# 1275468127/Medical-SAM2

Measured on AMD Instinct MI355X. Metric: slices/sec @1024^2 (Hiera-S), higher is better.
Workload: dtype bf16; 1 GPU; configs[1]: sam2_hiera_s 2D (train_2d SAM2 sub-sequence, forward), b=4 x 1024x1024 per GPU, 16-entry memory bank with 4 sampled memories per slice, one click per slice; forward_image -> memory_attention -> prompt encoder -> mask decoder -> memory encoder; hip_graph=True, weights=random name-keyed init

## Files before the change

include/msam2_hip.h:

```cpp
#ifndef MSAM2_HIP_H
#define MSAM2_HIP_H

#include <stddef.h>
#include <stdint.h>

#ifdef __cplusplus
extern "C" {
#endif

const char* msam2_last_error(void);

int msam2_version(void);

int msam2_operand_is_fp16(void);

int msam2_graph_begin(void* stream);

int msam2_graph_end(void* stream, void** graph_exec_out);

int msam2_graph_launch(void* graph_exec, void* stream);

int msam2_graph_destroy(void* graph_exec);

int msam2_event_create(void** ev);
// ... 185 lines not shown
int msam2_ln_mlp_residual_fwd(const float* x, int64_t T, int64_t dim, const float* ln_w, const float* ln_b, float eps, const void* w1, const float* b1, const void* w2p, const float* b2, float* out, void* stream);

int msam2_ln_mlp_residual_fwd_dual(const float* x, int64_t T, int64_t dim, const float* ln_w, const float* ln_b, float eps, const void* w1, const float* b1, const void* w2p, const float* b2, float* out, void* out16, void* stream);

size_t msam2_mask_stats_workspace_bytes(int64_t M);

int msam2_mask_stats(const float* logits, int64_t M, int64_t lh, int64_t lw, int64_t h, int64_t w, float thr, float thr_hi, float thr_lo, int* counts, int* boxes, void* workspace, size_t workspace_bytes, void* stream);

int msam2_mask_rle_runs(const float* logits, int64_t M, int64_t lh, int64_t lw, int64_t h, int64_t w, int64_t x0, int64_t y0, int64_t H, int64_t W, float thr, int* runs, void* stream);

int msam2_mask_rle(const float* logits, int64_t M, int64_t lh, int64_t lw, int64_t h, int64_t w, int64_t x0, int64_t y0, int64_t H, int64_t W, float thr, const int64_t* offsets, int* counts, void* stream);

size_t msam2_box_nms_workspace_bytes(int64_t K);

int msam2_box_nms(const float* boxes, const float* scores, int64_t K, float iou_thr, int64_t* keep, int* n_keep, void* workspace, size_t workspace_bytes, void* stream);

#ifdef __cplusplus
}
#endif
#endif
```

medical-sam2_amd/_lib.py:

```python
from __future__ import annotations

import ctypes
import os
import subprocess

_HERE = os.path.dirname(os.path.abspath(__file__))
LIB_PATH = os.environ.get("MSAM2_LIB_PATH") or os.path.join(_HERE, "libmsam2_hip.so")

c_p = ctypes.c_void_p
c_i = ctypes.c_int
c_l = ctypes.c_int64
c_f = ctypes.c_float
c_z = ctypes.c_size_t

SIGNATURES = {
    "msam2_version": (c_i, []),
    "msam2_last_error": (ctypes.c_char_p, []),
    "msam2_operand_is_fp16": (c_i, []),
    "msam2_gemm": (c_i, [c_p, c_l, c_p, c_l, c_p, c_p, c_p, c_l, c_i, c_l, c_p, c_l, c_i, c_l, c_l, c_l, c_i, c_p]),
    "msam2_gemm_pool2x2": (c_i, [c_p, c_l, c_p, c_l, c_p, c_p, c_l, c_l, c_l, c_l, c_l, c_l, c_p]),
    "msam2_gemm_qkv_pool2x2": (c_i, [c_p, c_l, c_p, c_l, c_p, c_p, c_l, c_p, c_l, c_l, c_l, c_l, c_l, c_l, c_l, c_p]),
    "msam2_gemm_tokens": (c_i, [c_p, c_l, c_p, c_l, c_p, c_l, c_p, c_p, c_l, c_p, c_l, c_i, c_l, c_l, c_l, c_i, c_p]),
    "msam2_gemm_rope": (c_i, [c_p, c_l, c_p, c_l, c_p, c_p, c_l, c_l, c_l, c_l, c_p, c_p, c_l, c_l, c_l, c_l, c_l, c_p]),
    "msam2_ln_mlp_residual_supported": (c_i, [c_l]),
# ... 89 lines not shown
    "msam2_box_nms": (c_i, [c_p, c_p, c_l, c_f, c_p, c_p, c_p, c_z, c_p]),
    "msam2_cc_workspace_bytes": (c_z, [c_l, c_l, c_l]),
    "msam2_cc_label": (c_i, [c_p, c_p, c_p, c_l, c_l, c_l, c_p, c_z, c_p]),
    "msam2_fill_holes_workspace_bytes": (c_z, [c_l, c_l, c_l]),
    "msam2_fill_holes": (c_i, [c_p, c_l, c_l, c_l, c_i, c_p, c_z, c_p]),
    "msam2_fill_components": (c_i, [c_p, c_l, c_l, c_l, c_i, c_f, c_i, c_f, c_p, c_z, c_p]),
    "msam2_image_prep": (c_i, [c_p, c_p, c_l, c_l, c_l, ctypes.POINTER(c_f), ctypes.POINTER(c_f), c_p]),
    "msam2_graph_begin": (c_i, [c_p]),
    "msam2_graph_end": (c_i, [c_p, ctypes.POINTER(c_p)]),
    "msam2_graph_launch": (c_i, [c_p, c_p]),
    "msam2_graph_destroy": (c_i, [c_p]),
    "msam2_event_create": (c_i, [ctypes.POINTER(c_p)]),
    "msam2_event_record": (c_i, [c_p, c_p]),
    "msam2_event_elapsed_ms": (c_i, [c_p, c_p, ctypes.POINTER(c_f)]),
    "msam2_event_destroy": (c_i, [c_p]),
}


def build(force: bool = False) -> str:
    if force and os.path.exists(LIB_PATH):
        os.remove(LIB_PATH)
    subprocess.check_call(["make", "-s", "-C", os.path.join(_HERE, "csrc")])
    return LIB_PATH


_lib = None


def lib() -> ctypes.CDLL:
    global _lib
# ... 22 lines not shown
```

medical-sam2_amd/modeling/common.py:

```python
from __future__ import annotations

from typing import Callable, Dict, Sequence, Tuple

import torch

from .. import ops

OP16, F32 = ops.OP16, torch.float32


class WeightCache:

    def __init__(self):
        self._c: Dict[str, Tuple[tuple, object]] = {}
        self._casts: Dict[str, torch.Tensor] = {}

    @staticmethod
    def _sig(params: Sequence[torch.Tensor]) -> tuple:
        return tuple((p.data_ptr(), p._version, str(p.device), p.dtype) for p in params)

    def get(self, key: str, params: Sequence[torch.Tensor], build: Callable[[], object], cast_of: torch.Tensor = None):
        sig = self._sig(params)
        hit = self._c.get(key)
        if hit is None or hit[0] != sig:
# ... 101 lines not shown
```

medical-sam2_amd/modeling/encoder.py:

```python
from __future__ import annotations

from typing import List, Optional, Tuple

import torch
import torch.nn as nn

from .. import ops
from .common import OP16, F32, WeightCache, nchw_view, to_bf16, tokens_of, v_f32, w_bf16
from .position import PositionEmbeddingSine


import os as _os
_POOL_GEMM = _os.environ.get("MSAM2_NO_POOL_GEMM") is None
_QPOOL_GEMM = _os.environ.get("MSAM2_NO_QPOOL_GEMM") is None
_FUSED_MLP = _os.environ.get("MSAM2_NO_FUSED_MLP") is None
_FUSED_PATCH = _os.environ.get("MSAM2_NO_FUSED_PATCH") is None


class PatchEmbed(nn.Module):

    def __init__(self, kernel_size=(7, 7), stride=(4, 4), padding=(3, 3), in_chans: int = 3, embed_dim: int = 768):
        super().__init__()
        assert tuple(kernel_size) == (7, 7) and tuple(stride) == (4, 4) and tuple(padding) == (3, 3) and in_chans == 3, \
            "the HIP path implements the 7x7/4/3 RGB patch embedding used by every SAM2 config"
# ... 126 lines not shown
            out = torch.zeros(3, heads, Dp, dtype=F32, device=b.device)
            out[:, :, :D] = b
            return out.reshape(-1).contiguous()

        def proj_w():
            w = a.proj.weight.detach().reshape(dim_out, heads, D)
            out = torch.zeros(dim_out, heads, Dp, dtype=w.dtype, device=w.device)
            out[:, :, :D] = w
            return out.reshape(dim_out, heads * Dp).to(OP16).contiguous()

        if Dp == D:
            return D, Dp, w_bf16(wc, "qkvw", a.qkv.weight), v_f32(wc, "qkvb", a.qkv.bias), w_bf16(wc, "ow", a.proj.weight)
        return (D, Dp, wc.get("qkvw_p", [a.qkv.weight], qkv_w), wc.get("qkvb_p", [a.qkv.bias], qkv_b),
                wc.get("ow_p", [a.proj.weight], proj_w))

    def run(self, t: torch.Tensor, B: int, H: int, W: int, emit16: bool = False) -> Tuple[torch.Tensor, int, int]:
        self.out16 = None
        wc, a = self._wc, self.attn
        heads, dim_out = a.num_heads, self.dim_out
        D, Dp, qkv_w, qkv_b, proj_w = self._packed_attn_weights()
        width = heads * Dp
        scale = 1.0 / (D ** 0.5)
        xn = ops.layernorm(t, v_f32(wc, "n1w", self.norm1.weight), v_f32(wc, "n1b", self.norm1.bias), 1e-6)
        pool = self.q_stride is not None
        if self.dim != dim_out:
            if _POOL_GEMM and pool and B * H * W >= 256 and H % 2 == 0 and W % 2 == 0:
                shortcut = ops.gemm_pool2x2(xn, w_bf16(wc, "pw", self.proj.weight), v_f32(wc, "pb", self.proj.bias), B, H, W)
            else:
                shortcut = ops.gemm(xn, w_bf16(wc, "pw", self.proj.weight), v_f32(wc, "pb", self.proj.bias), out_dtype=F32)
                if pool:
                    shortcut = ops.maxpool2x2(shortcut, B, H, W)
        else:
            shortcut = t
        if _POOL_GEMM and _QPOOL_GEMM and pool and B * H * W >= 256 and H % 2 == 0 and W % 2 == 0 and width % 32 == 0:
            qkv, qp = ops.gemm_qkv_pool2x2(xn, qkv_w, qkv_b, B, H, W, width)
        else:
            qkv = ops.gemm(xn, qkv_w, qkv_b)
            qp = ops.maxpool2x2(qkv[:, :width], B, H, W) if pool else None
        Hq, Wq = (H // 2, W // 2) if pool else (H, W)
        if self.window_size > 0:
            o = ops.window_attention(qkv, B, H, W, heads, self.window_size, qkv_b, q_pooled=qp, scale=scale)
        else:
            v5 = qkv.view(B, H * W, 3, heads, Dp)
            q = (qp.view(B, Hq * Wq, heads, Dp) if pool else v5[:, :, 0]).permute(0, 2, 1, 3)
            o = ops.attention(q, v5[:, :, 1].permute(0, 2, 1, 3), v5[:, :, 2].permute(0, 2, 1, 3), scale=scale)
            o = o.permute(0, 2, 1, 3).reshape(B * Hq * Wq, width)
        t = ops.gemm(o, proj_w, v_f32(wc, "ob", a.proj.bias), residual=shortcut, out_dtype=F32)
        mlp = self.mlp
        if (_FUSED_MLP and ops.ln_mlp_residual_supported(dim_out) and mlp.num_layers == 2 and mlp._act_code == ops.ACT_GELU
                and mlp.layers[0].out_features == 4 * dim_out and Hq * Wq >= 1024):
            w2p = mlp._wc.get("w1p", [mlp.layers[1].weight], lambda: ops.mlp_fused_permute_w2(mlp.layers[1].weight.detach().to(OP16).contiguous()))
            t = ops.ln_mlp_residual(t, v_f32(wc, "n2w", self.norm2.weight), v_f32(wc, "n2b", self.norm2.bias), 1e-6,
                                    w_bf16(mlp._wc, "w0", mlp.layers[0].weight), v_f32(mlp._wc, "b0", mlp.layers[0].bias), w2p,
                                    v_f32(mlp._wc, "b1", mlp.layers[1].bias), also16=emit16)
            if emit16:
                t, self.out16 = t
            return t, Hq, Wq
        xn2 = ops.layernorm(t, v_f32(wc, "n2w", self.norm2.weight), v_f32(wc, "n2b", self.norm2.bias), 1e-6)
        t = self.mlp.run(xn2, residual=t, out_dtype=F32)
        return t, Hq, Wq

    def forward(self, x: torch.Tensor) -> torch.Tensor:
        B, H, W, C = x.shape
        t, h, w = self.run(x.to(F32).reshape(B * H * W, C).contiguous(), B, H, W)
        return t.reshape(B, h, w, -1)


class Hiera(nn.Module):

    def __init__(self, embed_dim: int = 96, num_heads: int = 1, drop_path_rate: float = 0.0, q_pool: int = 3,
                 q_stride: Tuple[int, int] = (2, 2), stages: Tuple[int, ...] = (2, 3, 16, 3), dim_mul: float = 2.0,
                 head_mul: float = 2.0, window_pos_embed_bkg_spatial_size: Tuple[int, int] = (14, 14),
                 window_spec: Tuple[int, ...] = (8, 4, 14, 7), global_att_blocks: Tuple[int, ...] = (12, 16, 20),
                 return_interm_layers=True):
        super().__init__()
# ... 28 lines not shown
        self._wc = WeightCache()

    def _pos_tokens(self, h: int, w: int) -> torch.Tensor:
        return self._wc.get(f"pos{h}x{w}", [self.pos_embed, self.pos_embed_window],
                            lambda: ops.hiera_pos_embed(self.pos_embed.detach().float(), self.pos_embed_window.detach().float(), h, w))

    def _get_pos_embed(self, hw: Tuple[int, int]) -> torch.Tensor:
        h, w = hw
        return self._pos_tokens(h, w).reshape(1, h, w, -1)

    def forward(self, x: torch.Tensor) -> List[torch.Tensor]:
        B, _, S, _ = x.shape
        h = w = S // 4
        t = self.patch_embed.tokens(x, self._pos_tokens(h, w))
        outputs = []
        for i, blk in enumerate(self.blocks):
            is_out = i == self.stage_ends[-1] or (i in self.stage_ends and self.return_interm_layers)
            t, h, w = blk.run(t, B, h, w, emit16=is_out)
            if is_out:
                v = nchw_view(t, B, h, w)
                v._op16_tokens, blk.out16 = blk.out16, None
                outputs.append(v)
        return outputs


class FpnNeck(nn.Module):

    def __init__(self, position_encoding: nn.Module, d_model: int, backbone_channel_list: List[int], kernel_size: int = 1,
                 stride: int = 1, padding: int = 0, fpn_interp_model: str = "bilinear", fuse_type: str = "sum",
                 fpn_top_down_levels: Optional[List[int]] = None):
        super().__init__()
        assert kernel_size == 1 and stride == 1 and padding == 0, "lateral convs are 1x1 in every SAM2 config"
        assert fpn_interp_model == "nearest" and fuse_type == "sum", "HIP path implements the YAML's nearest/sum top-down fusion"
# ... 60 lines not shown
```

medical-sam2_amd/modeling/memory.py:

```python
from __future__ import annotations

import copy
import math
from typing import Optional, Tuple

import torch
import torch.nn as nn

from .. import ops
from .common import OP16, F32, WeightCache, attn_splits, nchw_view, to_bf16, tokens_of, v_f32, w_bf16
from .encoder import MLP


import os as _os
_FUSED_ROPE = _os.environ.get("MSAM2_NO_FUSED_ROPE") is None
_FOLD_V = _os.environ.get("MSAM2_NO_VALUE_FOLD") is None
_BATCH_K_PROJ = _os.environ.get("MSAM2_BATCHED_KPROJ") is not None


class LayerNorm2d(nn.Module):

    def __init__(self, num_channels: int, eps: float = 1e-6) -> None:
        super().__init__()
        self.weight = nn.Parameter(torch.ones(num_channels))
        self.bias = nn.Parameter(torch.zeros(num_channels))
# ... 13 lines not shown
        self.kv_in_dim = kv_in_dim if kv_in_dim is not None else embedding_dim
        self.internal_dim = embedding_dim // downsample_rate
        self.num_heads = num_heads
        assert self.internal_dim % num_heads == 0, "num_heads must divide embedding_dim."
        self.q_proj = nn.Linear(embedding_dim, self.internal_dim)
        self.k_proj = nn.Linear(self.kv_in_dim, self.internal_dim)
        self.v_proj = nn.Linear(self.kv_in_dim, self.internal_dim)
        self.out_proj = nn.Linear(self.internal_dim, embedding_dim)
        self.dropout_p = dropout
        self._wc = WeightCache()

    def proj(self, which: str, x_bf16: torch.Tensor) -> torch.Tensor:
        lin = getattr(self, which + "_proj")
        return ops.gemm(x_bf16, w_bf16(self._wc, which + "w", lin.weight), v_f32(self._wc, which + "b", lin.bias))

    def out(self, o_bf16: torch.Tensor, residual: Optional[torch.Tensor], out_dtype=F32) -> torch.Tensor:
        return ops.gemm(o_bf16, w_bf16(self._wc, "ow", self.out_proj.weight), v_f32(self._wc, "ob", self.out_proj.bias),
                        residual=residual, out_dtype=out_dtype)

    def core(self, q: torch.Tensor, k: torch.Tensor, v: torch.Tensor) -> torch.Tensor:
        B, Lq, C = q.shape
        D = C // self.num_heads
        if D in (16, 32):
            return ops.attention_small(q, k, v, self.num_heads).reshape(B * Lq, C)
        H = self.num_heads
        sp = lambda t: t.view(B, t.shape[1], H, D).permute(0, 2, 1, 3)
        o = ops.attention(sp(q), sp(k), sp(v), splits=attn_splits(B, H, Lq, k.shape[1]))
        return o.permute(0, 2, 1, 3).reshape(B * Lq, C)

    def forward(self, q: torch.Tensor, k: torch.Tensor, v: torch.Tensor) -> torch.Tensor:
        assert not (self.training and self.dropout_p > 0.0), "attention dropout (train mode) is outside the forward hot path"
        B, Lq, _ = q.shape
        f = lambda t, n: self.proj(n, to_bf16(t.reshape(-1, t.shape[-1]).contiguous())).view(B, t.shape[1], -1)
# ... 35 lines not shown
        tiles_total = -(-valid_keys // 32)
        tiles_per = -(-tiles_total // eff)
        k0 = min(share[0] * tiles_per * 32, valid_keys)
        k1 = min(share[1] * tiles_per * 32, valid_keys)
        r0, r1 = (k0 // n_pos) * n_pos, min(-(-k1 // n_pos) * n_pos, Nk)
        kk = torch.empty(B, Nk, self.internal_dim, dtype=OP16, device=mem_k.device)
        if r1 > r0:
            n_rope = max(0, min(Nk - n_ptr_tokens, r1) - r0)
            for b in range(B):
                self.proj_rope("k", mem_k[b, r0:r1], 1, r1 - r0, n_rope, tab, out=kk[b, r0:r1])
        return kk

    def folds_values(self) -> bool:
        return _FOLD_V and self.kv_in_dim == 64 and self.internal_dim == 256 and self.num_heads == 1

    def out_folded(self, o64: torch.Tensor, residual: Optional[torch.Tensor], out_dtype=F32) -> torch.Tensor:
        ps = [self.out_proj.weight, self.out_proj.bias, self.v_proj.weight, self.v_proj.bias]
        w = self._wc.get("ovw", ps, lambda: (self.out_proj.weight.detach().float() @ self.v_proj.weight.detach().float()).to(OP16).contiguous())
        b = self._wc.get("ovb", ps, lambda: (self.out_proj.weight.detach().float() @ self.v_proj.bias.detach().float()
                                             + self.out_proj.bias.detach().float()).contiguous())
        return ops.gemm(o64, w, b, residual=residual, out_dtype=out_dtype)

    def core_folded(self, q: torch.Tensor, k: torch.Tensor, mem_v: torch.Tensor, key_count: Optional[torch.Tensor] = None) -> torch.Tensor:
        from .. import parallel
        B, Lq, C = q.shape
        Lk = k.shape[1]
        q4, k4, v4 = (q.view(B, Lq, 1, C).permute(0, 2, 1, 3), k.view(B, Lk, 1, C).permute(0, 2, 1, 3),
                      mem_v.reshape(B, Lk, 1, 64).permute(0, 2, 1, 3))
        splits = attn_splits(B, 1, Lq, Lk)
        kvs = parallel.current_kv_split()
        eff = ops.attention_effective_splits(Lk, splits) if kvs is not None else 1
        if eff > 1:
            ws = ops.attention_workspace(B, 1, Lq, 64, eff, q.device)
            s0, s1 = kvs.share(eff)
            ops.attention_kv64_partial(q4, k4, v4, splits=eff, split_begin=s0, split_count=s1 - s0, workspace=ws, key_count=key_count)
# ... 32 lines not shown
        self.linear1 = nn.Linear(d_model, dim_feedforward)
        self.dropout = nn.Dropout(dropout)
        self.linear2 = nn.Linear(dim_feedforward, d_model)
        self.norm1, self.norm2, self.norm3 = nn.LayerNorm(d_model), nn.LayerNorm(d_model), nn.LayerNorm(d_model)
        self.dropout1, self.dropout2, self.dropout3 = nn.Dropout(dropout), nn.Dropout(dropout), nn.Dropout(dropout)
        self.activation_str = activation
        self.pos_enc_at_attn = pos_enc_at_attn
        self.pos_enc_at_cross_attn_queries = pos_enc_at_cross_attn_queries
        self.pos_enc_at_cross_attn_keys = pos_enc_at_cross_attn_keys
        self._wc = WeightCache()

    def _ln(self, name: str, x: torch.Tensor) -> torch.Tensor:
        n = getattr(self, name)
        return ops.layernorm(x, v_f32(self._wc, name + "w", n.weight), v_f32(self._wc, name + "b", n.bias), n.eps)

    def run(self, x: torch.Tensor, mem_k: torch.Tensor, mem_v: torch.Tensor, B: int, L: int, n_ptr_tokens: int,
            key_count: Optional[torch.Tensor] = None, kk: Optional[torch.Tensor] = None) -> torch.Tensor:
        wc, sa, ca = self._wc, self.self_attn, self.cross_attn_image
        C = self.d_model
        Nk = mem_k.shape[1]
        tab = sa.table(L, x.device)
        t = self._ln("norm1", x)
        w_qkv = w_bf16(wc, "sqkv", sa.q_proj.weight, sa.k_proj.weight, sa.v_proj.weight)
        b_qkv = v_f32(wc, "sqkvb", sa.q_proj.bias, sa.k_proj.bias, sa.v_proj.bias)
        fused_rope = _FUSED_ROPE and B * L >= 256 and L >= 128 and sa.num_heads == 1 and B * L * 3 * C * 4 < 2 ** 31
        if fused_rope:
            qkv = ops.gemm_rope(t, w_qkv, b_qkv, tab, rope_cols=2 * C, head_dim=C, rows_per_batch=L, n_rope=L).view(B, L, 3 * C)
        else:
            qkv = ops.gemm(t, w_qkv, b_qkv).view(B, L, 3 * C)
        q, k, v = qkv[:, :, :C], qkv[:, :, C:2 * C], qkv[:, :, 2 * C:]
        if not fused_rope:
            ops.rope_(q, L, tab)
            ops.rope_(k, L, tab)
        x = sa.out(sa.core(q, k, v), x)
        t = self._ln("norm2", x)
        q = ca.proj_rope("q", t, B, L, L, tab)
        from .. import parallel
        kvs = parallel.current_kv_split()
        eff = ops.attention_effective_splits(Nk, attn_splits(B, 1, L, Nk)) if (kvs is not None and ca.folds_values()) else 1
        valid = Nk if key_count is None else (kvs.host_key_count if kvs is not None else None)
        if kk is not None:
            pass
        elif eff > 1 and valid is not None and (Nk - n_ptr_tokens) % tab[0].shape[0] == 0:
            kk = ca.proj_rope_key_range(mem_k, n_ptr_tokens, tab, int(valid), eff, kvs.share(eff))
        else:
            kk = ca.proj_rope("k", mem_k.reshape(B * Nk, -1), B, Nk, Nk - n_ptr_tokens, tab)
        if ca.folds_values():
            x = ca.out_folded(ca.core_folded(q, kk, mem_v, key_count), x)
        else:
            if key_count is not None:
                raise RuntimeError("a padded memory bank (key_count) needs the value-folded cross-attention (MSAM2_NO_VALUE_FOLD is set)")
            vv = ca.proj("v", mem_v.reshape(B * Nk, -1)).view(B, Nk, C)
            x = ca.out(ca.core(q, kk, vv), x)
        t = self._ln("norm3", x)
        h = ops.gemm(t, w_bf16(wc, "f1", self.linear1.weight), v_f32(wc, "f1b", self.linear1.bias), act=ops.ACT_RELU)
        return ops.gemm(h, w_bf16(wc, "f2", self.linear2.weight), v_f32(wc, "f2b", self.linear2.bias), residual=x, out_dtype=F32)

    def forward(self, tgt, memory, pos: Optional[torch.Tensor] = None, query_pos: Optional[torch.Tensor] = None,
                num_k_exclude_rope: int = 0) -> torch.Tensor:
        assert not self.training or self.dropout_value == 0.0, \
            "train-mode dropout runs through MemoryAttention.forward / training.* (backward.memory_attention_forward_saved), not a bare layer"
        B, L, C = tgt.shape
        mem_k = ops.add_cast(memory, pos, 1.0, OP16)
        mem_v = ops.add_cast(memory, None, 1.0, OP16)
        x = ops.add_cast(tgt, None, 1.0, F32).reshape(B * L, C)
        return self.run(x, mem_k, mem_v, B, L, num_k_exclude_rope).view(B, L, C)


class MemoryAttention(nn.Module):

    def __init__(self, d_model: int, pos_enc_at_input: bool, layer: nn.Module, num_layers: int, batch_first: bool = True):
# ... 56 lines not shown
        if ag.active(self) and key_count is None:
            pos = curr_pos if (curr_pos is not None and self.pos_enc_at_input) else torch.zeros_like(curr)
            return ag.memory_attention(self, curr, pos, memory, memory_pos, num_obj_ptr_tokens)
        drop = self.next_dropout()
        if drop is not None:
            from .. import backward as bwd
            assert key_count is None, "padded memory banks are an inference-path feature"
            zero = torch.zeros_like(curr) if curr_pos is None or not self.pos_enc_at_input else curr_pos
            return bwd.memory_attention_forward_saved(self, curr, zero, memory, memory_pos, num_obj_ptr_tokens, dropout=drop)[0]
        use_pos = self.pos_enc_at_input and curr_pos is not None
        x = ops.add_cast(curr.transpose(0, 1), curr_pos.transpose(0, 1) if use_pos else None, 0.1, F32).reshape(B * L, C)
        mem_bf = memory.transpose(0, 1)
        mem_k = ops.add_cast(mem_bf, memory_pos.transpose(0, 1), 1.0, OP16)
        mem_v = ops.add_cast(mem_bf, None, 1.0, OP16)
        kk_all = self._project_all_keys(mem_k, B, L, num_obj_ptr_tokens)
        for i, layer in enumerate(self.layers):
            x = layer.run(x, mem_k, mem_v, B, L, num_obj_ptr_tokens, key_count, None if kk_all is None else kk_all[:, :, i])
        y = ops.layernorm(x, v_f32(self._wc, "nw", self.norm.weight), v_f32(self._wc, "nb", self.norm.bias), self.norm.eps,
                          out_dtype=F32)
        return y.view(B, L, C).transpose(0, 1)


class MaskDownSampler(nn.Module):

    def __init__(self, embed_dim=256, kernel_size=4, stride=4, padding=0, total_stride=16, activation=nn.GELU):
        super().__init__()
        assert (kernel_size, stride, padding, total_stride) == (3, 2, 1, 16) and activation is nn.GELU, \
            "HIP path implements the YAML's k3/s2/p1 mask down-sampler"
        num_layers = int(math.log2(total_stride) // math.log2(stride))
        self.encoder = nn.Sequential()
        cin = 1
        for _ in range(num_layers):
            cout = cin * (stride ** 2)
            self.encoder.append(nn.Conv2d(cin, cout, kernel_size=kernel_size, stride=stride, padding=padding))
# ... 110 lines not shown
```

medical-sam2_amd/ops.py:

```python
from __future__ import annotations

import ctypes
import math
from typing import Optional, Tuple

import torch

from ._lib import check, lib

OP16 = torch.float16 if lib().msam2_operand_is_fp16() else torch.bfloat16

F32 = torch.float32
ACT_NONE, ACT_GELU, ACT_RELU, ACT_SIGMOID = 0, 1, 2, 3


def _stream() -> int:
    return torch.cuda.current_stream().cuda_stream


def _p(t: Optional[torch.Tensor]):
    return None if t is None else t.data_ptr()


def _is_bf16(t: torch.Tensor) -> int:
# ... 81 lines not shown
    _req(out.dtype == OP16 and out.shape == (M, N) and out.stride(1) == 1, "gemm_rope: out must be 16-bit [M, N] row-major")
    check(lib().msam2_gemm_rope(_p(a), a.stride(0), _p(w), w.stride(0), _p(bias), _p(out), out.stride(0), M, N, K, _p(cs), _p(sn),
                                rope_cols, head_dim, rows_per_batch, n_rope, cs.shape[0], _stream()))
    return out


def layernorm(x: torch.Tensor, weight: torch.Tensor, bias: torch.Tensor, eps: float, *, act: int = ACT_NONE,
              out_dtype: torch.dtype = OP16) -> torch.Tensor:
    C = x.shape[-1]
    x2 = x.reshape(-1, C)
    _req(x2.stride(1) == 1, "layernorm input rows must be contiguous")
    y = torch.empty(x2.shape, dtype=out_dtype, device=x.device)
    check(lib().msam2_layernorm(_p(x2), _is_bf16(x2), x2.stride(0), _p(weight), _p(bias), _p(y), _is_bf16(y), y.stride(0),
                                x2.shape[0], C, eps, act, _stream()))
    return y.reshape(x.shape)


def layernorm_dual(x: torch.Tensor, weight: torch.Tensor, bias: torch.Tensor, eps: float):
    C = x.shape[-1]
    x2 = x.reshape(-1, C)
    _req(x2.dtype == F32 and x2.stride(1) == 1 and C % 4 == 0, "layernorm_dual: fp32 rows, C % 4 == 0")
    y = torch.empty(x2.shape, dtype=F32, device=x.device)
    y16 = torch.empty(x2.shape, dtype=OP16, device=x.device)
    check(lib().msam2_layernorm_dual(_p(x2), x2.stride(0), _p(weight), _p(bias), _p(y), y.stride(0), _p(y16), y16.stride(0), x2.shape[0], C, eps,
                                     _stream()))
    return y.reshape(x.shape), y16.reshape(x.shape)


def ln_mlp_residual_supported(dim: int) -> bool:
    return bool(lib().msam2_ln_mlp_residual_supported(dim))
# ... 577 lines not shown
```

Measured before the change: 673.2 slices/s.

## Fuse output-projection GEMM with residual add and following LayerNorm

Adds a HIP kernel in which one workgroup owns full 256- or 384-column rows, so it can finish a GEMM with bias and residual and then apply LayerNorm in the epilogue. It writes both the fp32 residual stream and the normalized 16-bit or fp32 output. The kernel is wired into Hiera block projections, MLP outputs feeding the next block's norm1, and memory-attention out-projections and FFN outputs chained into the next layer's norms. This removes a separate LayerNorm launch and a round trip of the activation through memory. In exchange, each workgroup covers only 64 rows with full N, which limits GEMM tiling flexibility and occupancy.

```diff
diff --git a/include/msam2_hip.h b/include/msam2_hip.h
--- a/include/msam2_hip.h
+++ b/include/msam2_hip.h
@@ -223,6 +223,8 @@
 size_t msam2_box_nms_workspace_bytes(int64_t K);
 
 int msam2_box_nms(const float* boxes, const float* scores, int64_t K, float iou_thr, int64_t* keep, int* n_keep, void* workspace, size_t workspace_bytes, void* stream);
+
+int msam2_gemm_ln(const void* A, int64_t lda, const void* W, int64_t ldw, const float* bias, const float* residual, int64_t ldr, float* C, int64_t ldc, const float* ln_weight, const float* ln_bias, float eps, void* Y, int y_is_16bit, int64_t ldy, int64_t M, int64_t N, int64_t K, void* stream);
 
 #ifdef __cplusplus
 }
diff --git a/medical-sam2_amd/_lib.py b/medical-sam2_amd/_lib.py
--- a/medical-sam2_amd/_lib.py
+++ b/medical-sam2_amd/_lib.py
@@ -127,6 +127,7 @@
     "msam2_event_record": (c_i, [c_p, c_p]),
     "msam2_event_elapsed_ms": (c_i, [c_p, c_p, ctypes.POINTER(c_f)]),
     "msam2_event_destroy": (c_i, [c_p]),
+    "msam2_gemm_ln": (c_i, [c_p, c_l, c_p, c_l, c_p, c_p, c_l, c_p, c_l, c_p, c_p, c_f, c_p, c_i, c_l, c_l, c_l, c_l, c_p]),
 }
 
 
diff --git a/medical-sam2_amd/csrc/gemm_ln.hip b/medical-sam2_amd/csrc/gemm_ln.hip
--- /dev/null
+++ b/medical-sam2_amd/csrc/gemm_ln.hip
@@ -0,0 +1,250 @@
+#include "common.h"
+
+struct GemmLnParams {
+  const op16* A;
+  const op16* W;
+  const float* bias;
+  const float* R;
+  float* C;
+  const float* gamma;
+  const float* beta;
+  void* Y;
+  int64_t lda, ldw, ldr, ldc, ldy;
+  int M, K;
+  float eps;
+};
+
+constexpr int GLN_BM = 64, GLN_BK = 32, GLN_NST = 4;
+template <int N>
+struct GemmLnShape {
+  static constexpr int A_BYTES = GLN_BM * GLN_BK * 2;
+  static constexpr int STAGE_BYTES = (GLN_BM + N) * GLN_BK * 2;
+  static constexpr int SLD = N + 8;
+  static constexpr int TILE_BYTES = GLN_BM * SLD * 4;
+  static constexpr int LDS_BYTES = GLN_NST * STAGE_BYTES > TILE_BYTES ? GLN_NST * STAGE_BYTES : TILE_BYTES;
+  static_assert(LDS_BYTES <= 160 * 1024, "one workgroup per CU: 160 KiB of LDS");
+};
+
+template <int CHUNKS, typename VI>
+__device__ __forceinline__ void ln_row16_stats(const VI (&t)[CHUNKS], float (&v)[CHUNKS][4], int l16, int nch, int C, float eps, float& mean,
+                                               float& rstd) {
+#pragma clang fp contract(off)
+  float s = 0.f;
+#pragma unroll
+  for (int j = 0; j < CHUNKS; ++j) {
+    const bool in = l16 + 16 * j < nch;
+#pragma unroll
+    for (int e = 0; e < 4; ++e) {
+      v[j][e] = in ? (float)t[j][e] : 0.f;
+      s += v[j][e];
+    }
+  }
+#pragma unroll
+  for (int o = 8; o > 0; o >>= 1) s += __shfl_xor(s, o, 64);
+  mean = s / C;
+  float q = 0.f;
+#pragma unroll
+  for (int j = 0; j < CHUNKS; ++j) {
+    const bool in = l16 + 16 * j < nch;
+#pragma unroll
+    for (int e = 0; e < 4; ++e) {
+      const float d = in ? v[j][e] - mean : 0.f;
+      q = __builtin_fmaf(d, d, q);
+    }
+  }
+#pragma unroll
+  for (int o = 8; o > 0; o >>= 1) q += __shfl_xor(q, o, 64);
+  rstd = 1.0f / sqrtf(q / C + eps);
+}
+__device__ __forceinline__ float ln_affine(float v, float mean, float rstd, float w, float b) {
+#pragma clang fp contract(off)
+  return __builtin_fmaf((v - mean) * rstd, w, b);
+}
+
+template <int N, typename TY>
+__global__ __launch_bounds__(256, 1) void gemm_ln_kernel(GemmLnParams p) {
+#if defined(__HIP_DEVICE_COMPILE__)
+  typedef GemmLnShape<N> S;
+  constexpr int BM = GLN_BM, BK = GLN_BK, NST = GLN_NST;
+  constexpr int FM = 2, FN = N / 128, TN = N / 4;
+  constexpr int PW = N / 64;
+  constexpr int G = 1 + PW;
+  constexpr int CH = N / 64;
+  static_assert(N % 128 == 0 && G * (NST - 1) <= 63, "vmcnt is a 6-bit counter");
+  extern __shared__ __attribute__((aligned(1024))) unsigned char lds[];
+  const int tid = threadIdx.x;
+  const int wave = __builtin_amdgcn_readfirstlane(tid >> 6), lane = tid & 63;
+  const int r = lane & 31, h = lane >> 5;
+  const int64_t m0 = (int64_t)blockIdx.x * BM;
+
+  const auto a_rsrc = raw_rsrc(p.A);
+  const auto w_rsrc = raw_rsrc(p.W);
+  unsigned offA_src, offW_src[PW];
+  {
+    const int row = Img64::piece_row(wave, lane);
+    offA_src = (unsigned)(min(m0 + row, (int64_t)p.M - 1) * p.lda * 2 + Img64::src_chunk(row, lane) * 16);
+  }
+#pragma unroll
+  for (int i = 0; i < PW; ++i) {
+    const int row = Img64::piece_row(wave * PW + i, lane);
+    offW_src[i] = (unsigned)(row * p.ldw * 2 + Img64::src_chunk(row, lane) * 16);
+  }
+  auto issue = [&](int kt) {
+    unsigned char* base = lds + (kt % NST) * S::STAGE_BYTES;
+    const unsigned so = (unsigned)kt * BK * 2;
+    glds16_asm(a_rsrc, base + wave * 1024, offA_src, so);
+    unsigned char* wb = base + S::A_BYTES + wave * PW * 1024;
+#pragma unroll
+    for (int i = 0; i + 3 <= PW; i += 3) glds16x3_asm(w_rsrc, wb + i * 1024, offW_src[i], offW_src[i + 1], offW_src[i + 2], so);
+#pragma unroll
+    for (int i = PW - PW % 3; i < PW; ++i) glds16_asm(w_rsrc, wb + i * 1024, offW_src[i], so);
+  };
+
+  f32x16 acc[FM][FN];
+  zero_acc(acc);
+
+  int offA[FM][2], offB[FN][2];
+#pragma unroll
+  for (int i = 0; i < FM; ++i) {
+    const int ra = i * 32 + r;
+#pragma unroll
+    for (int ks = 0; ks < 2; ++ks) offA[i][ks] = ra * Img64::ROW_BYTES + (((2 * ks + h) ^ Img64::swz(ra)) << 4);
+  }
+#pragma unroll
+  for (int j = 0; j < FN; ++j) {
+    const int rb = wave * TN + j * 32 + r;
+#pragma unroll
+    for (int ks = 0; ks < 2; ++ks) offB[j][ks] = S::A_BYTES + rb * Img64::ROW_BYTES + (((2 * ks + h) ^ Img64::swz(rb)) << 4);
+  }
+
+  const int nk = p.K / BK;
+  auto wait_groups = [&](int younger) {
+    if (younger >= 3) wait_vmcnt<3 * G>();
+    else if (younger == 2) wait_vmcnt<2 * G>();
+    else if (younger == 1) wait_vmcnt<G>();
+    else wait_vmcnt<0>();
+  };
+  auto load_frags = [&](const unsigned char* sb, int ks, op16x8 (&af)[FM], op16x8 (&bfr)[FN]) {
+#pragma unroll
+    for (int i = 0; i < FM; ++i) af[i] = *reinterpret_cast<const op16x8*>(sb + offA[i][ks]);
+#pragma unroll
+    for (int j = 0; j < FN; ++j) bfr[j] = *reinterpret_cast<const op16x8*>(sb + offB[j][ks]);
+  };
+  auto mma = [&](const op16x8 (&af)[FM], const op16x8 (&bfr)[FN]) {
+#pragma unroll
+    for (int i = 0; i < FM; ++i)
+#pragma unroll
+      for (int j = 0; j < FN; ++j) acc[i][j] = MSAM2_MFMA_32x32x16(af[i], bfr[j], acc[i][j], 0, 0, 0);
+  };
+#pragma unroll
+  for (int i = 0; i < NST; ++i)
+    if (nk > i) issue(i);
+  wait_groups(min(nk, NST) - 1);
+  __builtin_amdgcn_s_barrier();
+  op16x8 a0[FM], b0[FN], a1[FM], b1[FN];
+  load_frags(lds, 0, a0, b0);
+  for (int kt = 0; kt < nk; ++kt) {
+    const unsigned char* sb = lds + (kt % NST) * S::STAGE_BYTES;
+    load_frags(sb, 1, a1, b1);
+    mma(a0, b0);
+    if (kt + 1 < nk) {
+      wait_groups(min(nk - 2 - kt, NST - 2));
+      asm volatile("s_waitcnt lgkmcnt(0)" ::: "memory");
+      __builtin_amdgcn_s_barrier();
+      if (kt + NST < nk) issue(kt + NST);
+      load_frags(lds + ((kt + 1) % NST) * S::STAGE_BYTES, 0, a0, b0);
+    }
+    mma(a1, b1);
+  }
+
+  const int l16 = tid & 15, rp = tid >> 4;
+  f32x4 rv[4][CH], b4[CH], g4[CH], be4[CH];
+#pragma unroll
+  for (int ps = 0; ps < 4; ++ps) {
+    const float* rr = p.R + min(m0 + ps * 16 + rp, (int64_t)p.M - 1) * p.ldr;
+#pragma unroll
+    for (int j = 0; j < CH; ++j) rv[ps][j] = *reinterpret_cast<const f32x4*>(rr + (l16 + 16 * j) * 4);
+  }
+#pragma unroll
+  for (int j = 0; j < CH; ++j) {
+    b4[j] = p.bias ? *reinterpret_cast<const f32x4*>(p.bias + (l16 + 16 * j) * 4) : f32x4{0.f, 0.f, 0.f, 0.f};
+    g4[j] = *reinterpret_cast<const f32x4*>(p.gamma + (l16 + 16 * j) * 4);
+    be4[j] = *reinterpret_cast<const f32x4*>(p.beta + (l16 + 16 * j) * 4);
+  }
+  __builtin_amdgcn_s_barrier();
+  float* tile = reinterpret_cast<float*>(lds);
+#pragma unroll
+  for (int i = 0; i < FM; ++i)
+#pragma unroll
+    for (int j = 0; j < FN; ++j)
+#pragma unroll
+      for (int e = 0; e < 16; ++e) tile[(i * 32 + (e & 3) + 8 * (e >> 2) + 4 * h) * S::SLD + wave * TN + j * 32 + r] = acc[i][j][e];
+  __syncthreads();
+#pragma unroll
+  for (int ps = 0; ps < 4; ++ps) {
+    const int row = ps * 16 + rp;
+    const int64_t m = m0 + row;
+    const bool live = m < p.M;
+    f32x4 tv[CH];
+#pragma unroll
+    for (int j = 0; j < CH; ++j) {
+      const f32x4 t = *reinterpret_cast<const f32x4*>(tile + row * S::SLD + (l16 + 16 * j) * 4);
+#pragma unroll
+      for (int e = 0; e < 4; ++e) {
+        const float x = t[e] + b4[j][e];
+        tv[j][e] = x + rv[ps][j][e];
+      }
+      if (live) *reinterpret_cast<f32x4*>(p.C + m * p.ldc + (l16 + 16 * j) * 4) = tv[j];
+    }
+    float v[CH][4];
+    float mean, rstd;
+    ln_row16_stats<CH>(tv, v, l16, N / 4, N, p.eps, mean, rstd);
+    if (live) {
+      TY* yr = reinterpret_cast<TY*>(p.Y) + m * p.ldy;
+#pragma unroll
+      for (int j = 0; j < CH; ++j) {
+        typedef __attribute__((ext_vector_type(4))) TY VO;
+        VO o;
+#pragma unroll
+        for (int e = 0; e < 4; ++e) o[e] = f2out<TY>(ln_affine(v[j][e], mean, rstd, g4[j][e], be4[j][e]));
+        *reinterpret_cast<VO*>(yr + (l16 + 16 * j) * 4) = o;
+      }
+    }
+  }
+#endif
+}
+
+template <int N, typename TY>
+static void launch_gemm_ln(const GemmLnParams& p, hipStream_t s) {
+  ensure_dyn_lds<gemm_ln_kernel<N, TY>>(GemmLnShape<N>::LDS_BYTES);
+  hipLaunchKernelGGL((gemm_ln_kernel<N, TY>), dim3(cdiv(p.M, GLN_BM)), dim3(256), GemmLnShape<N>::LDS_BYTES, s, p);
+}
+
+extern "C" int msam2_gemm_ln(const void* A, int64_t lda, const void* W, int64_t ldw, const float* bias, const float* residual, int64_t ldr,
+                             float* C, int64_t ldc, const float* ln_weight, const float* ln_bias, float eps, void* Y, int y_is_16bit,
+                             int64_t ldy, int64_t M, int64_t N, int64_t K, void* stream) {
+  MSAM2_REQUIRE(A && W && residual && C && ln_weight && ln_bias && Y, "gemm_ln: null tensor");
+  MSAM2_REQUIRE(N == 256 || N == 384, "gemm_ln: N=%lld unsupported (a workgroup owns whole rows of 256 or 384 columns)", (long long)N);
+  MSAM2_REQUIRE(K >= 64 && K <= 2048 && K % 32 == 0, "gemm_ln: K=%lld unsupported (a multiple of 32 in [64, 2048])", (long long)K);
+  MSAM2_REQUIRE(M > 0 && M < (1ll << 31), "gemm_ln: M=%lld out of range", (long long)M);
+  MSAM2_REQUIRE(lda % 8 == 0 && ldw % 8 == 0 && lda >= K && ldw >= K, "gemm_ln: lda, ldw must be multiples of 8 (16-byte rows) and >= K");
+  MSAM2_REQUIRE(ldr % 4 == 0 && ldc % 4 == 0 && ldy % 4 == 0 && ldr >= N && ldc >= N && ldy >= N,
+                "gemm_ln: ldr, ldc, ldy must be multiples of 4 and >= N");
+  MSAM2_REQUIRE((((uintptr_t)A | (uintptr_t)W | (uintptr_t)residual | (uintptr_t)C | (uintptr_t)ln_weight | (uintptr_t)ln_bias |
+                  (uintptr_t)bias) & 15) == 0 && ((uintptr_t)Y & (y_is_16bit ? 7 : 15)) == 0,
+                "gemm_ln: A, W, bias, residual, C, LayerNorm weight / bias must be 16-byte aligned, Y 8-byte (16-bit) or 16-byte (fp32)");
+  MSAM2_REQUIRE(M * lda * 2 < (1ll << 31) && N * ldw * 2 < (1ll << 31), "gemm_ln: A / W beyond the 32-bit offsets of the LDS-DMA");
+  GemmLnParams p;
+  p.A = (const op16*)A; p.W = (const op16*)W; p.bias = bias; p.R = residual; p.C = C; p.gamma = ln_weight; p.beta = ln_bias; p.Y = Y;
+  p.lda = lda; p.ldw = ldw; p.ldr = ldr; p.ldc = ldc; p.ldy = ldy;
+  p.M = (int)M; p.K = (int)K; p.eps = eps;
+  hipStream_t s = (hipStream_t)stream;
+  if (N == 384) {
+    if (y_is_16bit) launch_gemm_ln<384, op16>(p, s);
+    else launch_gemm_ln<384, float>(p, s);
+  } else {
+    if (y_is_16bit) launch_gemm_ln<256, op16>(p, s);
+    else launch_gemm_ln<256, float>(p, s);
+  }
+  return msam2_check_launch("gemm_ln");
+}
diff --git a/medical-sam2_amd/modeling/common.py b/medical-sam2_amd/modeling/common.py
--- a/medical-sam2_amd/modeling/common.py
+++ b/medical-sam2_amd/modeling/common.py
@@ -1,5 +1,6 @@
 from __future__ import annotations
 
+import os as _os
 from typing import Callable, Dict, Sequence, Tuple
 
 import torch
@@ -7,6 +8,13 @@
 from .. import ops
 
 OP16, F32 = ops.OP16, torch.float32
+
+_GEMM_LN = _os.environ.get("MSAM2_NO_GEMM_LN") is None
+_GEMM_LN_MIN_M = 16384
+
+
+def use_gemm_ln(M: int, N: int, K: int) -> bool:
+    return _GEMM_LN and M >= _GEMM_LN_MIN_M and ops.gemm_ln_supported(M, N, K)
 
 
 class WeightCache:
diff --git a/medical-sam2_amd/modeling/encoder.py b/medical-sam2_amd/modeling/encoder.py
--- a/medical-sam2_amd/modeling/encoder.py
+++ b/medical-sam2_amd/modeling/encoder.py
@@ -6,7 +6,7 @@
 import torch.nn as nn
 
 from .. import ops
-from .common import OP16, F32, WeightCache, nchw_view, to_bf16, tokens_of, v_f32, w_bf16
+from .common import OP16, F32, WeightCache, nchw_view, to_bf16, tokens_of, use_gemm_ln, v_f32, w_bf16
 from .position import PositionEmbeddingSine
 
 
@@ -164,14 +164,16 @@
         return (D, Dp, wc.get("qkvw_p", [a.qkv.weight], qkv_w), wc.get("qkvb_p", [a.qkv.bias], qkv_b),
                 wc.get("ow_p", [a.proj.weight], proj_w))
 
-    def run(self, t: torch.Tensor, B: int, H: int, W: int, emit16: bool = False) -> Tuple[torch.Tensor, int, int]:
+    def run(self, t: torch.Tensor, B: int, H: int, W: int, emit16: bool = False, *, xn: Optional[torch.Tensor] = None,
+            next_norm: Optional[nn.LayerNorm] = None):
         self.out16 = None
         wc, a = self._wc, self.attn
         heads, dim_out = a.num_heads, self.dim_out
         D, Dp, qkv_w, qkv_b, proj_w = self._packed_attn_weights()
         width = heads * Dp
         scale = 1.0 / (D ** 0.5)
-        xn = ops.layernorm(t, v_f32(wc, "n1w", self.norm1.weight), v_f32(wc, "n1b", self.norm1.bias), 1e-6)
+        if xn is None:
+            xn = ops.layernorm(t, v_f32(wc, "n1w", self.norm1.weight), v_f32(wc, "n1b", self.norm1.bias), 1e-6)
         pool = self.q_stride is not None
         if self.dim != dim_out:
             if _POOL_GEMM and pool and B * H * W >= 256 and H % 2 == 0 and W % 2 == 0:
@@ -195,20 +197,37 @@
             q = (qp.view(B, Hq * Wq, heads, Dp) if pool else v5[:, :, 0]).permute(0, 2, 1, 3)
             o = ops.attention(q, v5[:, :, 1].permute(0, 2, 1, 3), v5[:, :, 2].permute(0, 2, 1, 3), scale=scale)
             o = o.permute(0, 2, 1, 3).reshape(B * Hq * Wq, width)
-        t = ops.gemm(o, proj_w, v_f32(wc, "ob", a.proj.bias), residual=shortcut, out_dtype=F32)
         mlp = self.mlp
-        if (_FUSED_MLP and ops.ln_mlp_residual_supported(dim_out) and mlp.num_layers == 2 and mlp._act_code == ops.ACT_GELU
-                and mlp.layers[0].out_features == 4 * dim_out and Hq * Wq >= 1024):
+        fused_mlp = (_FUSED_MLP and ops.ln_mlp_residual_supported(dim_out) and mlp.num_layers == 2 and mlp._act_code == ops.ACT_GELU
+                     and mlp.layers[0].out_features == 4 * dim_out and Hq * Wq >= 1024)
+        T = B * Hq * Wq
+        xn2 = None
+        if not fused_mlp and use_gemm_ln(T, dim_out, width):
+            t, xn2 = ops.gemm_ln(o, proj_w, v_f32(wc, "ob", a.proj.bias), shortcut, v_f32(wc, "n2w", self.norm2.weight),
+                                 v_f32(wc, "n2b", self.norm2.bias), 1e-6)
+        else:
+            t = ops.gemm(o, proj_w, v_f32(wc, "ob", a.proj.bias), residual=shortcut, out_dtype=F32)
+        if fused_mlp:
             w2p = mlp._wc.get("w1p", [mlp.layers[1].weight], lambda: ops.mlp_fused_permute_w2(mlp.layers[1].weight.detach().to(OP16).contiguous()))
             t = ops.ln_mlp_residual(t, v_f32(wc, "n2w", self.norm2.weight), v_f32(wc, "n2b", self.norm2.bias), 1e-6,
                                     w_bf16(mlp._wc, "w0", mlp.layers[0].weight), v_f32(mlp._wc, "b0", mlp.layers[0].bias), w2p,
                                     v_f32(mlp._wc, "b1", mlp.layers[1].bias), also16=emit16)
             if emit16:
                 t, self.out16 = t
-            return t, Hq, Wq
-        xn2 = ops.layernorm(t, v_f32(wc, "n2w", self.norm2.weight), v_f32(wc, "n2b", self.norm2.bias), 1e-6)
-        t = self.mlp.run(xn2, residual=t, out_dtype=F32)
-        return t, Hq, Wq
+            return (t, Hq, Wq) if next_norm is None else (t, Hq, Wq, None)
+        if xn2 is None:
+            xn2 = ops.layernorm(t, v_f32(wc, "n2w", self.norm2.weight), v_f32(wc, "n2b", self.norm2.bias), 1e-6)
+        if next_norm is None:
+            return self.mlp.run(xn2, residual=t, out_dtype=F32), Hq, Wq
+        xn_next = None
+        hidden = mlp.layers[0].out_features
+        if (mlp.num_layers == 2 and not mlp.sigmoid_output and next_norm.normalized_shape == (dim_out,) and use_gemm_ln(T, dim_out, hidden)):
+            hdn = ops.gemm(xn2, w_bf16(mlp._wc, "w0", mlp.layers[0].weight), v_f32(mlp._wc, "b0", mlp.layers[0].bias), act=mlp._act_code)
+            t, xn_next = ops.gemm_ln(hdn, w_bf16(mlp._wc, "w1", mlp.layers[1].weight), v_f32(mlp._wc, "b1", mlp.layers[1].bias), t,
+                                     v_f32(wc, "nn1w", next_norm.weight), v_f32(wc, "nn1b", next_norm.bias), next_norm.eps)
+        else:
+            t = self.mlp.run(xn2, residual=t, out_dtype=F32)
+        return t, Hq, Wq, xn_next
 
     def forward(self, x: torch.Tensor) -> torch.Tensor:
         B, H, W, C = x.shape
@@ -267,9 +286,14 @@
         h = w = S // 4
         t = self.patch_embed.tokens(x, self._pos_tokens(h, w))
         outputs = []
+        xn = None
         for i, blk in enumerate(self.blocks):
             is_out = i == self.stage_ends[-1] or (i in self.stage_ends and self.return_interm_layers)
-            t, h, w = blk.run(t, B, h, w, emit16=is_out)
+            nxt = self.blocks[i + 1].norm1 if i + 1 < len(self.blocks) else None
+            if nxt is not None:
+                t, h, w, xn = blk.run(t, B, h, w, emit16=is_out, xn=xn, next_norm=nxt)
+            else:
+                (t, h, w), xn = blk.run(t, B, h, w, emit16=is_out, xn=xn), None
             if is_out:
                 v = nchw_view(t, B, h, w)
                 v._op16_tokens, blk.out16 = blk.out16, None
diff --git a/medical-sam2_amd/modeling/memory.py b/medical-sam2_amd/modeling/memory.py
--- a/medical-sam2_amd/modeling/memory.py
+++ b/medical-sam2_amd/modeling/memory.py
@@ -8,7 +8,7 @@
 import torch.nn as nn
 
 from .. import ops
-from .common import OP16, F32, WeightCache, attn_splits, nchw_view, to_bf16, tokens_of, v_f32, w_bf16
+from .common import use_gemm_ln, OP16, F32, WeightCache, attn_splits, nchw_view, to_bf16, tokens_of, v_f32, w_bf16
 from .encoder import MLP
 
 
@@ -52,9 +52,11 @@
         lin = getattr(self, which + "_proj")
         return ops.gemm(x_bf16, w_bf16(self._wc, which + "w", lin.weight), v_f32(self._wc, which + "b", lin.bias))
 
-    def out(self, o_bf16: torch.Tensor, residual: Optional[torch.Tensor], out_dtype=F32) -> torch.Tensor:
-        return ops.gemm(o_bf16, w_bf16(self._wc, "ow", self.out_proj.weight), v_f32(self._wc, "ob", self.out_proj.bias),
-                        residual=residual, out_dtype=out_dtype)
+    def out(self, o_bf16: torch.Tensor, residual: Optional[torch.Tensor], out_dtype=F32, ln=None):
+        w, b = w_bf16(self._wc, "ow", self.out_proj.weight), v_f32(self._wc, "ob", self.out_proj.bias)
+        if ln is not None:
+            return ops.gemm_ln(o_bf16, w, b, residual, *ln)
+        return ops.gemm(o_bf16, w, b, residual=residual, out_dtype=out_dtype)
 
     def core(self, q: torch.Tensor, k: torch.Tensor, v: torch.Tensor) -> torch.Tensor:
         B, Lq, C = q.shape
@@ -120,11 +122,13 @@
     def folds_values(self) -> bool:
         return _FOLD_V and self.kv_in_dim == 64 and self.internal_dim == 256 and self.num_heads == 1
 
-    def out_folded(self, o64: torch.Tensor, residual: Optional[torch.Tensor], out_dtype=F32) -> torch.Tensor:
+    def out_folded(self, o64: torch.Tensor, residual: Optional[torch.Tensor], out_dtype=F32, ln=None):
         ps = [self.out_proj.weight, self.out_proj.bias, self.v_proj.weight, self.v_proj.bias]
         w = self._wc.get("ovw", ps, lambda: (self.out_proj.weight.detach().float() @ self.v_proj.weight.detach().float()).to(OP16).contiguous())
         b = self._wc.get("ovb", ps, lambda: (self.out_proj.weight.detach().float() @ self.v_proj.bias.detach().float()
                                              + self.out_proj.bias.detach().float()).contiguous())
+        if ln is not None:
+            return ops.gemm_ln(o64, w, b, residual, *ln)
         return ops.gemm(o64, w, b, residual=residual, out_dtype=out_dtype)
 
     def core_folded(self, q: torch.Tensor, k: torch.Tensor, mem_v: torch.Tensor, key_count: Optional[torch.Tensor] = None) -> torch.Tensor:
@@ -187,13 +191,18 @@
         n = getattr(self, name)
         return ops.layernorm(x, v_f32(self._wc, name + "w", n.weight), v_f32(self._wc, name + "b", n.bias), n.eps)
 
+    def _ln_args(self, name: str):
+        n = getattr(self, name)
+        return v_f32(self._wc, name + "w", n.weight), v_f32(self._wc, name + "b", n.bias), n.eps
+
     def run(self, x: torch.Tensor, mem_k: torch.Tensor, mem_v: torch.Tensor, B: int, L: int, n_ptr_tokens: int,
-            key_count: Optional[torch.Tensor] = None, kk: Optional[torch.Tensor] = None) -> torch.Tensor:
+            key_count: Optional[torch.Tensor] = None, kk: Optional[torch.Tensor] = None, *, xn: Optional[torch.Tensor] = None,
+            next_norm=None, next_norm_dtype=OP16):
         wc, sa, ca = self._wc, self.self_attn, self.cross_attn_image
         C = self.d_model
         Nk = mem_k.shape[1]
         tab = sa.table(L, x.device)
-        t = self._ln("norm1", x)
+        t = xn if xn is not None else self._ln("norm1", x)
         w_qkv = w_bf16(wc, "sqkv", sa.q_proj.weight, sa.k_proj.weight, sa.v_proj.weight)
         b_qkv = v_f32(wc, "sqkvb", sa.q_proj.bias, sa.k_proj.bias, sa.v_proj.bias)
         fused_rope = _FUSED_ROPE and B * L >= 256 and L >= 128 and sa.num_heads == 1 and B * L * 3 * C * 4 < 2 ** 31
@@ -205,8 +214,12 @@
         if not fused_rope:
             ops.rope_(q, L, tab)
             ops.rope_(k, L, tab)
-        x = sa.out(sa.core(q, k, v), x)
-        t = self._ln("norm2", x)
+        o = sa.core(q, k, v)
+        if use_gemm_ln(B * L, C, o.shape[1]):
+            x, t = sa.out(o, x, ln=self._ln_args("norm2"))
+        else:
+            x = sa.out(o, x)
+            t = self._ln("norm2", x)
         q = ca.proj_rope("q", t, B, L, L, tab)
         from .. import parallel
         kvs = parallel.current_kv_split()
@@ -219,15 +232,29 @@
         else:
             kk = ca.proj_rope("k", mem_k.reshape(B * Nk, -1), B, Nk, Nk - n_ptr_tokens, tab)
         if ca.folds_values():
-            x = ca.out_folded(ca.core_folded(q, kk, mem_v, key_count), x)
+            o = ca.core_folded(q, kk, mem_v, key_count)
+            if use_gemm_ln(B * L, C, o.shape[1]):
+                x, t = ca.out_folded(o, x, ln=self._ln_args("norm3"))
+            else:
+                x, t = ca.out_folded(o, x), None
         else:
             if key_count is not None:
                 raise RuntimeError("a padded memory bank (key_count) needs the value-folded cross-attention (MSAM2_NO_VALUE_FOLD is set)")
             vv = ca.proj("v", mem_v.reshape(B * Nk, -1)).view(B, Nk, C)
-            x = ca.out(ca.core(q, kk, vv), x)
-        t = self._ln("norm3", x)
+            o = ca.core(q, kk, vv)
+            if use_gemm_ln(B * L, C, o.shape[1]):
+                x, t = ca.out(o, x, ln=self._ln_args("norm3"))
+            else:
+                x, t = ca.out(o, x), None
+        if t is None:
+            t = self._ln("norm3", x)
         h = ops.gemm(t, w_bf16(wc, "f1", self.linear1.weight), v_f32(wc, "f1b", self.linear1.bias), act=ops.ACT_RELU)
-        return ops.gemm(h, w_bf16(wc, "f2", self.linear2.weight), v_f32(wc, "f2b", self.linear2.bias), residual=x, out_dtype=F32)
+        w2, b2 = w_bf16(wc, "f2", self.linear2.weight), v_f32(wc, "f2b", self.linear2.bias)
+        if next_norm is None:
+            return ops.gemm(h, w2, b2, residual=x, out_dtype=F32)
+        if use_gemm_ln(B * L, C, h.shape[1]):
+            return ops.gemm_ln(h, w2, b2, x, *next_norm, ln_out_dtype=next_norm_dtype)
+        return ops.gemm(h, w2, b2, residual=x, out_dtype=F32), None
 
     def forward(self, tgt, memory, pos: Optional[torch.Tensor] = None, query_pos: Optional[torch.Tensor] = None,
                 num_k_exclude_rope: int = 0) -> torch.Tensor:
@@ -314,10 +341,14 @@
         mem_k = ops.add_cast(mem_bf, memory_pos.transpose(0, 1), 1.0, OP16)
         mem_v = ops.add_cast(mem_bf, None, 1.0, OP16)
         kk_all = self._project_all_keys(mem_k, B, L, num_obj_ptr_tokens)
+        xn = None
+        final = (v_f32(self._wc, "nw", self.norm.weight), v_f32(self._wc, "nb", self.norm.bias), self.norm.eps)
         for i, layer in enumerate(self.layers):
-            x = layer.run(x, mem_k, mem_v, B, L, num_obj_ptr_tokens, key_count, None if kk_all is None else kk_all[:, :, i])
-        y = ops.layernorm(x, v_f32(self._wc, "nw", self.norm.weight), v_f32(self._wc, "nb", self.norm.bias), self.norm.eps,
-                          out_dtype=F32)
+            last = i + 1 == len(self.layers)
+            nxt = final if last else self.layers[i + 1]._ln_args("norm1")
+            x, xn = layer.run(x, mem_k, mem_v, B, L, num_obj_ptr_tokens, key_count, None if kk_all is None else kk_all[:, :, i], xn=xn,
+                              next_norm=nxt, next_norm_dtype=F32 if last else OP16)
+        y = xn if xn is not None else ops.layernorm(x, *final, out_dtype=F32)
         return y.view(B, L, C).transpose(0, 1)
 
 
diff --git a/medical-sam2_amd/ops.py b/medical-sam2_amd/ops.py
--- a/medical-sam2_amd/ops.py
+++ b/medical-sam2_amd/ops.py
@@ -119,6 +119,34 @@
     check(lib().msam2_layernorm(_p(x2), _is_bf16(x2), x2.stride(0), _p(weight), _p(bias), _p(y), _is_bf16(y), y.stride(0),
                                 x2.shape[0], C, eps, act, _stream()))
     return y.reshape(x.shape)
+
+
+GEMM_LN_WIDTHS = (256, 384)
+
+
+def gemm_ln_supported(M: int, N: int, K: int) -> bool:
+    return N in GEMM_LN_WIDTHS and 64 <= K <= 2048 and K % 32 == 0 and M > 0
+
+
+def gemm_ln(a: torch.Tensor, w: torch.Tensor, bias: Optional[torch.Tensor], residual: torch.Tensor, ln_w: torch.Tensor, ln_b: torch.Tensor,
+            eps: float, *, ln_out_dtype: torch.dtype = OP16, out: Optional[torch.Tensor] = None,
+            ln_out: Optional[torch.Tensor] = None) -> Tuple[torch.Tensor, torch.Tensor]:
+    _req(a.dim() == 2 and w.dim() == 2 and a.shape[1] == w.shape[1], f"gemm_ln shapes {tuple(a.shape)} x {tuple(w.shape)}")
+    _req(a.dtype == OP16 and w.dtype == OP16 and a.stride(1) == 1 and w.stride(1) == 1, "gemm_ln operands: 16-bit, K-contiguous")
+    M, K = a.shape
+    N = w.shape[0]
+    _req(residual.dtype == F32 and residual.shape == (M, N) and residual.stride(1) == 1, "gemm_ln residual must be fp32 [M,N]")
+    _req(ln_w.dtype == F32 and ln_b.dtype == F32 and ln_w.shape == (N,) and ln_b.shape == (N,) and ln_w.is_contiguous()
+         and ln_b.is_contiguous(), "gemm_ln: LayerNorm weight / bias must be fp32 [N]")
+    if out is None:
+        out = torch.empty(M, N, dtype=F32, device=a.device)
+    if ln_out is None:
+        ln_out = torch.empty(M, N, dtype=ln_out_dtype, device=a.device)
+    _req(out.dtype == F32 and out.shape == (M, N) and out.stride(1) == 1, "gemm_ln out must be fp32 [M,N] row-major")
+    _req(ln_out.shape == (M, N) and ln_out.stride(1) == 1, "gemm_ln ln_out must be [M,N] row-major")
+    check(lib().msam2_gemm_ln(_p(a), a.stride(0), _p(w), w.stride(0), _p(bias), _p(residual), residual.stride(0), _p(out), out.stride(0),
+                              _p(ln_w), _p(ln_b), eps, _p(ln_out), _is_bf16(ln_out), ln_out.stride(0), M, N, K, _stream()))
+    return out, ln_out
 
 
 def layernorm_dual(x: torch.Tensor, weight: torch.Tensor, bias: torch.Tensor, eps: float):
```

After: 679.4 slices/s (median of 6 runs). Within noise of the previous version (+0.9%).
